# xmed-lab/NEURONS

Hardware: AMD Instinct MI355X
Metric: denoising frames/sec, 16f x 256^2 clip, 50 DDIM steps (higher is better)
Workload: dtype bf16; 1 GPU; BASELINE config 2: 1 clip(s) per call, (1,4,16,32,32) latent, 50 DDIM steps, CFG 8.5 (batch 2), SparseCtrl + temporal U-Net per step, random-init weights; clips_per_gpu=5, ddim_steps=50, hip_graph=True, output_finite=True, attention=bf16

## Files before the change

neurons_amd/csrc/engine.hip:

```cpp
#include "common.h"
#include "../../include/neurons_amd.h"

#include <cmath>
#include <cstdio>
#include <cstdlib>
#include <cstring>
#include <functional>
#include <map>
#include <memory>
#include <stdexcept>
#include <string>
#include <vector>

extern "C" {
int nr_launch_igemm(const NrGemmParams* pp, float* workspace, hipStream_t stream);
size_t nr_igemm_workspace_bytes(const NrGemmParams* pp);
size_t nr_lin160_stream_bytes(int N, int K);
int nr_lin160_eligible(const NrGemmParams* pp);
int nr_lin160_panel_rule(int Mp, int N, int K);
size_t nr_lin128q_stream_bytes(int N, int K);
int nr_launch_lin128q_w_pack(const bf16* w, int N, int K, bf16* stream, hipStream_t s);
int nr_launch_lin160_w_pack(const bf16* w, int N, int K, bf16* stream, hipStream_t s);
int nr_launch_lin160(const NrGemmParams* pp, const bf16* stream, hipStream_t s);
int nr_gn_workspace_floats(int nimg, int hw, int groups, int* pix_per_blk_out, int* nchunk_out);
int nr_launch_groupnorm(NrGnParams* pp, hipStream_t stream);
int nr_launch_layernorm(const bf16* x, int ldx, bf16* out, int ldo, int M, int C, const float* gamma, const float* beta,
                        float eps, const float* pe, int pe_hw, int pe_F, hipStream_t stream);
int nr_launch_attention(const NrAttnParams* pp, hipStream_t stream);
int nr_launch_conv_in_small(const float* s0, const float* s1, int c0, int c1, int src_batch, int nimg, int F, int H, int W,
                            const float* wT, const float* bias, const float* addend, int Cout, bf16* out, float in_scale,
                            float in_shift, hipStream_t stream);
int nr_launch_clip_embed(const int* ids, const float* tok, const float* pos, bf16* out, int M, int L, int C, int vocab,
                         hipStream_t stream);
int nr_launch_bf16_to_f32(const bf16* a, float* out, long long n, hipStream_t stream);
int nr_launch_gaussian_sample(const float* moments, const float* noise, float* out, int n, int zc, int hw, float scale,
                              hipStream_t stream);
int nr_launch_post_quant(const float* z, float scale, const float* Q, const float* qb, float* out, int nimg, int C, int hw,
                         hipStream_t stream);
int nr_launch_softmax_rows(const float* S, bf16* P, int rows, int L, float scale, hipStream_t stream);
int nr_launch_conv_out_small(const bf16* x, int Cin, int nimg, int F, int H, int W, const bf16* w, const float* bias,
                             int Cout, float* out, float out_mul, float out_add, int clamp01, hipStream_t stream);
int nr_launch_timestep_sincos(const float* t, int M, int dim, float* out, hipStream_t stream);
int nr_launch_linear_small(const float* x, int M, int K, const bf16* W, const float* b, int N, int in_act, int out_act,
                           float* y, const float* addend, hipStream_t stream);
int nr_launch_edm_cfg_euler(const float* net, const float* x, float* x_out, long long total, float scale, float sigma_q,
                            float sigma, float sigma_next, hipStream_t stream);
int nr_launch_cfg_combine(const float* eps, float* out, long long total, float guidance, hipStream_t stream);
int nr_launch_cfg_ddim_step(const float* eps, const float* x, float* x_out, long long total, float guidance, int do_cfg,
                            float sqrt_at, float sqrt_1mat, float sqrt_ap, float sqrt_1map, hipStream_t stream);
int nr_launch_add_bf16(const bf16* a, const bf16* b, bf16* out, long long n, hipStream_t stream);
int nr_launch_prior_p_sample(const float* pred, const float* pred_null, const float* x, const float* noise, float* x_out, float* x_start_out,
                             long long total, float cond_scale, int mode, int clamp, float sqrt_ac, float sqrt_1mac, float sqrt_recip_ac,
                             float sqrt_recipm1_ac, float coef1, float coef2, float sigma, hipStream_t stream);
int nr_launch_f32_to_bf16(const float* a, bf16* out, long long n, hipStream_t stream);
int nr_launch_add_bf16_multi(const NrAddMulti* p, hipStream_t stream);
int nr_launch_frame_gather(const bf16* src, bf16* dst, int B, int Fs, int Fd, long long frame_elems, const int* map, hipStream_t stream);
int nr_launch_ncfhw_to_nhwc(const float* src, bf16* dst, int B, int C, int F, int HW, hipStream_t stream);
int nr_launch_nhwc_to_ncfhw(const bf16* src, float* dst, int B, int C, int F, int HW, hipStream_t stream);
int nr_groupnorm_launches(const NrGnParams* p);
int nr_launch_fold_linear_pair(const float* w2, const float* w1, const float* b2, const float* b1, int C, int J, bf16* wc, float* bc,
                               hipStream_t stream);
int nr_smallm_eligible(const NrGemmParams* pp);
int nr_launch_smallm_w_pack(const void* w, void* out, int N, int K, hipStream_t stream);
size_t nr_xattn_wstream_bytes(void);
size_t nr_xattn_kvstream_bytes(int nctx);
int nr_xattn_fused_eligible(int C, int heads, int Lk, int hw, long long rows);
int nr_launch_xattn_w_pack(const bf16* wq, const bf16* wo, bf16* stream, hipStream_t s);
int nr_launch_xattn_kv_pack(const bf16* kv, int ldkv, int Lk, int nctx, bf16* stream, hipStream_t s);
int nr_launch_xattn_fused(bf16* t, int nimg, int hw, int img_per_ctx, int nctx, int Lk, const bf16* wstream, const bf16* kvstream, const float* gamma,
// ... 2785 lines not shown
}

extern "C" nr_status nr_op_gemm_ex(nr_stream stream, const void* a, int32_t lda, const void* w, const float* bias, const float* ln_c,
                                   float ln_eps, const float* rowvec, int32_t rowvec_div, int32_t rowvec_mod, int32_t rowvec_ld,
                                   const void* res, int32_t ldr, void* out, int32_t ldo, int32_t M, int32_t N, int32_t K, int32_t geglu,
                                   int32_t act, float out_scale) {
  NR_TRY
  NrGemmParams p;
  std::memset(&p, 0, sizeof(p));
  p.a0 = (const bf16*)a; p.c0 = K; p.lda0 = lda; p.H = p.W = p.OH = p.OW = 1; p.ksize = 1; p.stride = 1;
  p.w = (const bf16*)w; p.M = M; p.N = N; p.K = K; p.bias = bias; p.res = (const bf16*)res; p.ldr = ldr;
  p.out = (bf16*)out; p.ldo = ldo; p.out_scale = out_scale; p.geglu = geglu; p.act = act;
  p.rowvec = rowvec; p.rowvec_div = rowvec_div > 0 ? rowvec_div : 1; p.rowvec_mod = rowvec_mod; p.rowvec_ld = rowvec_ld;
  p.ln_c = ln_c; p.ln_eps = ln_eps;
  op_fragmajor(p, (hipStream_t)stream);
  LAUNCH_OK(nr_launch_igemm(&p, ln_c ? nullptr : op_workspace(p), (hipStream_t)stream));
  NR_CATCH
}

extern "C" nr_status nr_op_conv3x3(nr_stream stream, const void* x0, int32_t c0, const void* x1, int32_t c1, int32_t nimg,
                                   int32_t H, int32_t W, int32_t stride, int32_t ups, const void* w, const float* bias,
                                   const float* rowvec, int32_t rowvec_div, const void* res, void* out, int32_t Cout) {
  NR_TRY
  NrGemmParams p;
  std::memset(&p, 0, sizeof(p));
  p.a0 = (const bf16*)x0; p.c0 = c0; p.lda0 = c0; p.a1 = (const bf16*)x1; p.c1 = x1 ? c1 : 0; p.lda1 = c1;
  p.H = H; p.W = W;
  int OH = H, OW = W;
  if (ups) { OH *= 2; OW *= 2; }
  if (stride == 2) { OH = (OH - 1) / 2 + 1; OW = (OW - 1) / 2 + 1; }
  p.OH = OH; p.OW = OW; p.ksize = 3; p.stride = stride; p.ups = ups;
  p.w = (const bf16*)w; p.M = nimg * OH * OW; p.N = Cout; p.K = 9 * (p.c0 + p.c1);
  p.bias = bias; p.rowvec = rowvec; p.rowvec_div = rowvec_div > 0 ? rowvec_div : 1; p.rowvec_ld = Cout;
  p.res = (const bf16*)res; p.ldr = Cout; p.out = (bf16*)out; p.ldo = Cout; p.out_scale = 1.f;
  LAUNCH_OK(nr_launch_igemm(&p, op_workspace(p), (hipStream_t)stream));
  NR_CATCH
}

extern "C" nr_status nr_op_conv3x3_tap_inner(nr_stream stream, const void* x0, int32_t c0, int32_t nimg, int32_t H, int32_t W, const void* w,
                                             const float* bias, const float* rowvec, int32_t rowvec_div, const void* res, void* out,
                                             int32_t Cout) {
  NR_TRY
  NrGemmParams p;
  std::memset(&p, 0, sizeof(p));
  p.a0 = (const bf16*)x0; p.c0 = c0; p.lda0 = c0;
  p.H = H; p.W = W; p.OH = H; p.OW = W; p.ksize = 3; p.stride = 1; p.tap_inner = 1;
  p.w = (const bf16*)w; p.M = nimg * H * W; p.N = Cout; p.K = 9 * c0;
  p.bias = bias; p.rowvec = rowvec; p.rowvec_div = rowvec_div > 0 ? rowvec_div : 1; p.rowvec_ld = Cout;
  p.res = (const bf16*)res; p.ldr = Cout; p.out = (bf16*)out; p.ldo = Cout; p.out_scale = 1.f;
  LAUNCH_OK(nr_launch_igemm(&p, op_workspace(p), (hipStream_t)stream));
  NR_CATCH
}

extern "C" nr_status nr_op_groupnorm(nr_stream stream, const void* x0, int32_t c0, const void* x1, int32_t c1, int32_t nimg,
                                     int32_t hw, int32_t groups, const float* gamma, const float* beta, float eps,
                                     int32_t silu, float* partial_ws, void* out) {
  NR_TRY
  NrGnParams p;
  std::memset(&p, 0, sizeof(p));
  p.x0 = (const bf16*)x0; p.c0 = c0; p.ld0 = c0; p.x1 = (const bf16*)x1; p.c1 = x1 ? c1 : 0; p.ld1 = c1;
  p.nimg = nimg; p.hw = hw; p.groups = groups; p.partial = partial_ws; p.gamma = gamma; p.beta = beta; p.eps = eps;
  p.silu = silu; p.out = (bf16*)out; p.ldo = p.c0 + p.c1;
  LAUNCH_OK(nr_launch_groupnorm(&p, (hipStream_t)stream));
  NR_CATCH
}

extern "C" nr_status nr_op_layernorm(nr_stream stream, const void* x, void* out, int32_t M, int32_t C, const float* gamma,
                                     const float* beta, float eps, const float* pe, int32_t pe_hw, int32_t pe_F) {
  NR_TRY
  LAUNCH_OK(nr_launch_layernorm((const bf16*)x, C, (bf16*)out, C, M, C, gamma, beta, eps, pe, pe_hw > 0 ? pe_hw : 1,
                                pe_F > 0 ? pe_F : 1, (hipStream_t)stream));
  NR_CATCH
}

extern "C" nr_status nr_op_attention(nr_stream stream, int32_t mode, const void* qp, const void* kvp, void* outp,
                                     int32_t nimg, int32_t L, int32_t Lk, int32_t C, int32_t heads, int32_t frames,
                                     int32_t kv_div) {
  NR_TRY
  NrAttnParams p;
  std::memset(&p, 0, sizeof(p));
  const bf16* q = (const bf16*)qp; const bf16* kv = (const bf16*)kvp;
  const int fp8_flag = (mode & 8) ? 1 : 0;
  mode &= 7;
  p.heads = heads; p.d = C / heads; p.scale = 1.0f / std::sqrt((float)p.d); p.out = (bf16*)outp;
  if (mode == 0) {
    const int ld = 3 * C;
    p.q = q; p.k = q + C; p.v = q + 2 * C; p.nbatch = nimg; p.Lq = L; p.Lk = L; p.inner = 1; p.kv_inner = 1; p.kv_div = 1;
    p.q_outer = (long long)L * ld; p.q_seq = ld; p.kv_outer = p.q_outer; p.kv_seq = ld;
    p.o_outer = (long long)L * C; p.o_seq = C;
  } else if (mode == 1) {
    p.q = q; p.k = kv; p.v = kv + C; p.nbatch = nimg; p.Lq = L; p.Lk = Lk; p.inner = 1; p.kv_inner = 1; p.kv_div = kv_div;
    p.q_outer = (long long)L * C; p.q_seq = C; p.kv_outer = (long long)Lk * 2 * C; p.kv_seq = 2 * C;
    p.o_outer = (long long)L * C; p.o_seq = C;
  } else if (mode == 2) {
    const int ld = 3 * C, hw = L, F = frames;
    p.q = q; p.k = q + C; p.v = q + 2 * C; p.nbatch = (nimg / F) * hw; p.Lq = F; p.Lk = F; p.inner = hw; p.kv_inner = hw; p.kv_div = 1;
    p.q_outer = (long long)F * hw * ld; p.q_inner_stride = ld; p.q_seq = (long long)hw * ld;
    p.kv_outer = p.q_outer; p.kv_inner_stride = ld; p.kv_seq = p.q_seq;
    p.o_outer = (long long)F * hw * C; p.o_inner_stride = C; p.o_seq = (long long)hw * C;
  } else throw NrError(NR_ERR_ARG, "bad attention mode");
  p.fp8 = fp8_flag;
  LAUNCH_OK(nr_launch_attention(&p, (hipStream_t)stream));
  NR_CATCH
}

extern "C" nr_status nr_op_ff_fused(nr_stream stream, const void* t_dev, const void* x_dev, void* out_dev, int32_t M, int32_t C,
// ... 109 lines not shown
```

neurons_amd/csrc/gemm.hip:

```cpp
#include "common.h"
#include <cstdio>
#include <cstdlib>

namespace {

__device__ __attribute__((aligned(16))) const unsigned int nr_zero16[4] = {0u, 0u, 0u, 0u};

typedef const __attribute__((address_space(1))) void* gptr_t;
typedef __attribute__((address_space(3))) void* lptr_t;

__device__ __forceinline__ void glds16_asm(const void* src, unsigned lds_wave_base) {
  asm volatile("s_mov_b32 m0, %1\n\ts_nop 0\n\tglobal_load_lds_dwordx4 %0, off" : : "v"(src), "s"(lds_wave_base) : "memory", "m0");
}
__device__ __forceinline__ void glds16_builtin(const void* src, void* lds_wave_base) {
  __builtin_amdgcn_global_load_lds((gptr_t)src, (lptr_t)lds_wave_base, 16, 0, 0);
}
__device__ __forceinline__ unsigned lds_addr(const void* p) {
  return __builtin_amdgcn_readfirstlane((unsigned)(unsigned long long)(lptr_t)p);
}

template <int N> __device__ __forceinline__ void wait_vmcnt() {
  if constexpr (N == 0) asm volatile("s_waitcnt vmcnt(0)" ::: "memory");
  else if constexpr (N <= 63) asm volatile("s_waitcnt vmcnt(%0)" ::"n"(N) : "memory");
  else asm volatile("s_waitcnt vmcnt(0)" ::: "memory");
// ... 593 lines not shown
        hipLaunchKernelGGL((igemm_bf16_kernel<BM, BN, NS, WGM, WGN, false, true, true>), dim3(grid), dim3(64 * WGM * WGN), shm, stream, p, splitk, partial, m_fast);
      else
        hipLaunchKernelGGL((igemm_bf16_kernel<BM, BN, NS, WGM, WGN, false, false, true>), dim3(grid), dim3(64 * WGM * WGN), shm, stream, p, splitk, partial, m_fast);
      return 0;
    }
  }
  if (nk_slice >= adma_min)
    hipLaunchKernelGGL((igemm_bf16_kernel<BM, BN, NS, WGM, WGN, false, true>), dim3(grid), dim3(64 * WGM * WGN), shm, stream, p, splitk,
                       partial, m_fast);
  else
    hipLaunchKernelGGL((igemm_bf16_kernel<BM, BN, NS, WGM, WGN, false, false>), dim3(grid), dim3(64 * WGM * WGN), shm, stream, p, splitk,
                       partial, m_fast);
  return 0;
}

template <int BM, int BN, int WGM, int WGN>
int launch_tile(const NrGemmParams& p, unsigned grid, const Plan& pl, float* partial, int m_fast, hipStream_t stream) {
  constexpr size_t STAGE = (size_t)(BM + BN) * 64 * sizeof(bf16);
  constexpr bool FITS4 = 4 * STAGE <= 160 * 1024;
  if (pl.stages <= 2) return launch_cfg<BM, BN, 2, WGM, WGN>(p, grid, pl.splitk, partial, m_fast, stream);
  if (pl.stages == 3 || !FITS4) return launch_cfg<BM, BN, 3, WGM, WGN>(p, grid, pl.splitk, partial, m_fast, stream);
  if (pl.stages <= 4 || BM * BN > 64 * 64) return launch_cfg<BM, BN, 4, WGM, WGN>(p, grid, pl.splitk, partial, m_fast, stream);
  if (pl.stages <= 6) return launch_cfg<BM, BN, 6, WGM, WGN>(p, grid, pl.splitk, partial, m_fast, stream);
  return launch_cfg<BM, BN, 8, WGM, WGN>(p, grid, pl.splitk, partial, m_fast, stream);
}

void apply_override(const NrGemmParams& p, Plan& pl, int& m_fast) {
  const char* e = getenv("NR_IGEMM_FORCE");
  if (!e) return;
  if (const char* f = getenv("NR_IGEMM_FORCE_MAXM")) if (p.M > atoi(f)) return;
  if (const char* f = getenv("NR_IGEMM_FORCE_MINM")) if (p.M < atoi(f)) return;
  if (const char* f = getenv("NR_IGEMM_FORCE_KS")) if (p.ksize != atoi(f)) return;
  if (const char* f = getenv("NR_IGEMM_FORCE_N")) if (p.N != atoi(f)) return;
  if (const char* f = getenv("NR_IGEMM_FORCE_K")) if (p.K != atoi(f)) return;
  int bm = -1, bn = -1, sk = -1, st = -1, ord = -1, wv = -1;
  sscanf(e, "%d,%d,%d,%d,%d,%d", &bm, &bn, &sk, &st, &ord, &wv);
  if (bm > 0 && bn > 0) {
    const bool ok = (bm == 128 && (bn == 160 || bn == 128 || bn == 64)) || (bm == 64 && (bn == 64 || bn == 32 || bn == 160)) || (bm == 256 && (bn == 128 || bn == 160));
    if (ok && !(p.geglu && ((bn == 160 && !(bm == 128 && wv == 41)) || bn == 32))) { pl.bm = bm; pl.bn = bn; }
  }
  if (wv == 4 || wv == 8) pl.waves = wv;
  if (pl.bm == 256 && pl.bn == 128 && wv != 4) pl.waves = 8;
  if (pl.bn == 160 || pl.bm == 64) pl.waves = 4;
  if (wv == 41 && pl.bm == 128 && pl.bn == 160) pl.waves = 41;
  if (sk > 0 && !p.geglu) { const int nk = p.K / 64; pl.splitk = sk > nk ? nk : sk; }
  if (st >= 2 && st <= 8) pl.stages = st;
  if (ord >= 0) m_fast = ord;
}

}

extern "C" int nr_rowpanel_eligible(const NrGemmParams* pp);
extern "C" int nr_launch_rowpanel(const NrGemmParams* pp, hipStream_t stream);
extern "C" int nr_g8p_plan(const NrGemmParams* pp);
extern "C" int nr_launch_g8p(const NrGemmParams* pp, int m_fast, hipStream_t stream);
extern "C" int nr_smallm_eligible(const NrGemmParams* pp);
extern "C" int nr_launch_smallm(const NrGemmParams* pp, hipStream_t stream);

extern "C" size_t nr_igemm_workspace_bytes(const NrGemmParams* pp) {
  if (pp->out_f32 || pp->ln_c) return 0;
  if (nr_rowpanel_eligible(pp)) return 0;
  if (pp->w_fm) return 0;
  if (nr_g8p_plan(pp)) return 0;
  Plan pl = choose_plan(plan_view(*pp));
  int mf = 0;
  apply_override(*pp, pl, mf);
  return pl.splitk > 1 ? (size_t)pl.splitk * pp->M * pp->N * sizeof(float) : 0;
}

extern "C" int nr_launch_igemm(const NrGemmParams* pp, float* workspace, hipStream_t stream) {
  const NrGemmParams& p = *pp;
  const int Cin = p.c0 + p.c1;
  if (p.K == p.ksize * p.ksize * Cin && nr_rowpanel_eligible(pp)) return nr_launch_rowpanel(pp, stream);
  if (p.w_fm) return nr_launch_smallm(pp, stream);
  if (const int nt8 = nr_g8p_plan(pp)) {
    const double w_e = (double)p.N * p.K;
    const double a_e = (double)p.M * Cin;
    int mf = w_e > a_e ? 1 : 0;
    const int ntm_ = (p.M + 255) / 256, ntn_ = (p.N + 64 * nt8 - 1) / (64 * nt8);
    if (ntm_ >= 8 && ntn_ >= 4 && w_e >= 3.0e6) mf = 8;
    return nr_launch_g8p(pp, mf, stream);
  }
  if (p.K % 64 != 0 || Cin % 64 != 0 || p.N % 32 != 0) return 1;
  if (p.a1 && (p.c0 % 64 != 0)) return 2;
  if (p.K != p.ksize * p.ksize * Cin) return 3;
  if (p.ksize != 1 && p.ksize != 3) return 4;
  if (p.tap_inner && (p.ksize != 3 || p.stride != 1 || p.ups || p.pad_tl0 || p.a1)) return 5;
  Plan pl = choose_plan(plan_view(p));
  const double w_elems = (double)p.N * p.K;
  const double a_elems = (double)p.M * Cin * (p.ksize == 3 ? (p.stride == 2 ? 4.0 : (p.ups ? 0.25 : 1.0)) : 1.0);
  int m_fast = w_elems > a_elems ? 1 : 0;
  {
    static const bool grouped = !(getenv("NR_IGEMM_GROUPED") && getenv("NR_IGEMM_GROUPED")[0] == '0');
    const int ntm_ = (p.M + pl.bm - 1) / pl.bm, ntn_ = (p.N + pl.bn - 1) / pl.bn;
    static const double grouped_minw = getenv("NR_IGEMM_GROUPED_MINW") ? atof(getenv("NR_IGEMM_GROUPED_MINW")) : 3.0e6;
    if (grouped && ntm_ >= 8 && ntn_ >= 4 && w_elems >= grouped_minw) m_fast = 8;
  }
  apply_override(p, pl, m_fast);
  if (p.ln_c) {
    if (p.ksize != 1 || p.a1 || p.out_f32) return 8;
    pl.splitk = 1;
    if (pl.bn == 32) pl.bn = 64;
    const bool t64x160 = pl.bm == 64 && pl.bn == 160;
    if (!(pl.stages == 4 && (pl.bm * pl.bn <= 64 * 64 || (pl.bm == 128 && pl.bn == 64))) && pl.waves != 41 && !(t64x160 && pl.stages <= 3)) pl.stages = 2;
    if (pl.bm > 128) { pl.bm = 128; pl.bn = 128; pl.waves = 8; }
    if (pl.bn > 128 && !(pl.bm == 128 && pl.bn == 160 && pl.waves == 41) && !t64x160) { pl.bm = 128; pl.bn = 128; pl.waves = 8; }
    if (pl.waves == 41 && pl.stages > 4) pl.stages = 4;
  }
  if (p.out_f32) {
    if (p.geglu) return 7;
    pl.splitk = 1;
  }
  if (pl.splitk > 1 && !workspace) return 6;
  float* partial = p.out_f32 ? p.out_f32 : (pl.splitk > 1 ? workspace : nullptr);
  const unsigned grid = (unsigned)(((p.M + pl.bm - 1) / pl.bm) * ((p.N + pl.bn - 1) / pl.bn) * pl.splitk);
  int rc;
  if (pl.bm == 256 && pl.bn == 160) rc = launch_tile<256, 160, 2, 2>(p, grid, pl, partial, m_fast, stream);
  else if (pl.bm == 256 && pl.waves == 4) rc = launch_tile<256, 128, 2, 2>(p, grid, pl, partial, m_fast, stream);
  else if (pl.bm == 256) rc = launch_tile<256, 128, 4, 2>(p, grid, pl, partial, m_fast, stream);
  else if (pl.bm == 128 && pl.bn == 160 && pl.waves == 41)
    rc = pl.stages <= 3 ? launch_cfg<128, 160, 3, 4, 1>(p, grid, pl.splitk, partial, m_fast, stream)
                        : launch_cfg<128, 160, 4, 4, 1>(p, grid, pl.splitk, partial, m_fast, stream);
  else if (pl.bm == 128 && pl.bn == 160) rc = launch_tile<128, 160, 2, 2>(p, grid, pl, partial, m_fast, stream);
  else if (pl.bm == 128 && pl.bn == 128 && pl.waves == 8) rc = launch_tile<128, 128, 2, 4>(p, grid, pl, partial, m_fast, stream);
  else if (pl.bm == 128 && pl.bn == 128) rc = launch_tile<128, 128, 2, 2>(p, grid, pl, partial, m_fast, stream);
  else if (pl.bm == 128 && pl.bn == 64 && pl.waves == 8) rc = launch_tile<128, 64, 4, 2>(p, grid, pl, partial, m_fast, stream);
  else if (pl.bm == 128 && pl.bn == 64) rc = launch_tile<128, 64, 2, 2>(p, grid, pl, partial, m_fast, stream);
  else if (pl.bm == 64 && pl.bn == 160) rc = launch_tile<64, 160, 2, 2>(p, grid, pl, partial, m_fast, stream);
  else if (pl.bm == 64 && pl.bn == 32) rc = launch_tile<64, 32, 2, 2>(p, grid, pl, partial, m_fast, stream);
  else if (pl.bm == 64 && pl.bn == 64) rc = launch_tile<64, 64, 2, 2>(p, grid, pl, partial, m_fast, stream);
  else rc = 9;
  if (rc) return rc;
  if (pl.splitk > 1) {
    const long long total = (long long)p.M * (p.N / 4);
// ... 16 lines not shown
```

neurons_amd/csrc/gemm8p.hip:

```cpp
#include "common.h"
#include <cstdlib>

namespace {

__device__ __attribute__((aligned(16))) const unsigned int g8p_zero16[4] = {0u, 0u, 0u, 0u};
typedef __attribute__((address_space(3))) void* lptr_t;

__device__ __forceinline__ void glds16(const void* src, unsigned lds_wave_base) {
  asm volatile("s_mov_b32 m0, %1\n\ts_nop 0\n\tglobal_load_lds_dwordx4 %0, off" : : "v"(src), "s"(lds_wave_base) : "memory", "m0");
}
template <int N> __device__ __forceinline__ void wait_vm() { asm volatile("s_waitcnt vmcnt(%0)" ::"n"(N) : "memory"); }

__device__ __forceinline__ int fdiv_small(int a, int d) {
  int q = (int)((float)a * __builtin_amdgcn_rcpf((float)d));
  const int r = a - q * d;
  q += (r >= d ? 1 : 0) - (r < 0 ? 1 : 0);
  return q;
}
__device__ __forceinline__ size_t rowvec_row(const NrGemmParams& p, int m) {
  int r = m / p.rowvec_div;
  if (p.rowvec_mod) r %= p.rowvec_mod;
  return (size_t)r * p.rowvec_ld;
}

constexpr int G8_BM = 256, G8_BK = 64;

template <int NT, bool TAPI, int NPH = 4>
__global__ __launch_bounds__(512, 2) void g8p_kernel(NrGemmParams p_arg, int m_fast) {
  const NrGemmParams p = nr_pin_params(p_arg);
  m_fast = nr_pin(m_fast);
  constexpr int BN = 64 * NT, WN = 16 * NT;
  constexpr int A_BYTES = G8_BM * 128, B_BYTES = BN * 128, STAGE = A_BYTES + B_BYTES;
  static_assert(NPH == 4 || (NPH == 2 && NT <= 4), "phases per k-tile");
  extern __shared__ __attribute__((aligned(16))) char smem[];

  const int tid = threadIdx.x;
  const int lane = tid & 63;
  const int wave = __builtin_amdgcn_readfirstlane(tid >> 6);
  const int g = wave >> 2, wn = wave & 3;
  const int ntn = (p.N + BN - 1) / BN, ntm = (p.M + G8_BM - 1) / G8_BM;
  int bid;
  {
    const int nwg = gridDim.x, orig = blockIdx.x;
    const int q = nwg >> 3, r = nwg & 7, xcd = orig & 7, local = orig >> 3;
    bid = (xcd < r ? xcd * (q + 1) : r * (q + 1) + (xcd - r) * q) + local;
  }
  int bm, bn;
  if (m_fast >= 2) {
    const int G = m_fast;
    const int band = fdiv_small(bid, G * ntn);
    const int first = band * G;
    const int gsz = min(G, ntm - first);
    const int r = bid - band * G * ntn;
    bn = fdiv_small(r, gsz);
    bm = first + r - bn * gsz;
  } else if (m_fast) { bn = fdiv_small(bid, ntm); bm = bid - bn * ntm; } else { bm = fdiv_small(bid, ntn); bn = bid - bm * ntn; }
  const int m0 = bm * G8_BM, n0 = bn * BN;

  const int lr = lane >> 3, lp = lane & 7;
  const unsigned lchunk_b = (unsigned)((lp ^ lr) << 4);
  const char* zsrc = reinterpret_cast<const char*>(g8p_zero16);

  unsigned a_off[4];
  unsigned a_msk = 0, a_msk3 = 0;
  int a_m[4];
#pragma unroll
  for (int j = 0; j < 4; ++j) {
    const int m = m0 + 8 * (16 * g + 4 * wn + j) + lr;
    const bool ok = m < p.M;
    a_m[j] = ok ? m : 0;
    if constexpr (TAPI) {
      const int ohw = p.OH * p.OW;
      const int n = fdiv_small(a_m[j], ohw);
      const int r = a_m[j] - n * ohw;
      const int oy = fdiv_small(r, p.OW), ox = r - oy * p.OW;
      a_off[j] = (unsigned)((((size_t)n * p.H + oy) * p.W + ox) * (size_t)p.lda0 * sizeof(bf16)) + lchunk_b;
      unsigned msk = 0;
#pragma unroll
      for (int t = 0; t < 9; ++t) {
        const int iy = oy + t / 3 - 1, ix = ox + t % 3 - 1;
        if (ok && iy >= 0 && iy < p.H && ix >= 0 && ix < p.W) msk |= 1u << t;
      }
      if (j < 3) a_msk |= msk << (9 * j);
      else a_msk3 = msk;
    } else {
      a_off[j] = (unsigned)((size_t)a_m[j] * (size_t)p.lda0 * sizeof(bf16)) + lchunk_b;
      if (ok) a_msk |= 1u << j;
    }
  }
  unsigned w_off[NT];
  unsigned w_msk = 0;
#pragma unroll
  for (int j = 0; j < NT; ++j) {
    const int n = n0 + 8 * (NT * wave + j) + lr;
    const bool ok = n < p.N;
    w_off[j] = (unsigned)((size_t)(ok ? n : 0) * (size_t)p.K * sizeof(bf16)) + lchunk_b;
    if (ok) w_msk |= 1u << j;
  }

  const int nk = p.K / G8_BK;
  const unsigned lds0 = __builtin_amdgcn_readfirstlane((unsigned)(unsigned long long)(lptr_t)smem);
  const unsigned lds_a = lds0 + (unsigned)((16 * g + 4 * wn) * 1024);
  const unsigned lds_w = lds0 + (unsigned)A_BYTES + (unsigned)(NT * wave * 1024);

  auto a_base = [&](int kt, int& tap) -> const char* {
    if constexpr (TAPI) {
      const int c64 = kt / 9;
      tap = kt - 9 * c64;
      const int ky = tap / 3, kx = tap - 3 * ky;
      const long long delta = ((long long)(ky - 1) * p.W + (kx - 1)) * p.lda0 * (long long)sizeof(bf16);
      return reinterpret_cast<const char*>(p.a0 + c64 * G8_BK) + delta;
    } else {
      tap = 0;
      const int c = kt * G8_BK;
      return c < p.c0 ? reinterpret_cast<const char*>(p.a0 + c) : reinterpret_cast<const char*>(p.a1 + (c - p.c0));
    }
  };
  int a_src = 0;
  auto a_select_source = [&](int kt) {
    if constexpr (!TAPI) {
      const int want = (p.c1 > 0 && kt * G8_BK >= p.c0) ? 1 : 0;
      if (want != a_src) {
        a_src = want;
        const int ld = want ? p.lda1 : p.lda0;
#pragma unroll
        for (int j = 0; j < 4; ++j) a_off[j] = (unsigned)((size_t)a_m[j] * (size_t)ld * sizeof(bf16)) + lchunk_b;
      }
    }
  };
  auto issue_a = [&](const char* base, int tap, int stage, int j) {
    bool ok;
    if constexpr (TAPI) ok = ((j < 3 ? (a_msk >> (9 * j)) : a_msk3) >> tap) & 1u;
    else ok = (a_msk >> j) & 1u;
    const char* src = ok ? base + a_off[j] : zsrc;
    glds16(src, lds_a + (unsigned)(stage * STAGE + j * 1024));
  };
  auto issue_w = [&](int kt, int stage, int j) {
    const char* base = reinterpret_cast<const char*>(p.w) + (size_t)kt * (G8_BK * sizeof(bf16));
    const char* src = ((w_msk >> j) & 1u) ? base + w_off[j] : zsrc;
    glds16(src, lds_w + (unsigned)(stage * STAGE + j * 1024));
  };

  f32x4 acc[NT][8];
#pragma unroll
  for (int i = 0; i < NT; ++i)
#pragma unroll
    for (int j = 0; j < 8; ++j) acc[i][j] = f32x4{0.f, 0.f, 0.f, 0.f};

  const int fr = lane & 15, fg = lane >> 4;
  const unsigned frag0 = (unsigned)(fr * 128 + ((fg ^ (fr & 7)) << 4));
  const unsigned xrow = (unsigned)(g * 128 * 128), wrow = (unsigned)(A_BYTES + wn * WN * 128);

  {
    int tap;
    a_select_source(0);
    const char* ab = a_base(0, tap);
#pragma unroll
    for (int j = 0; j < 4; ++j) issue_a(ab, tap, 0, j);
#pragma unroll
    for (int j = 0; j < NT; ++j) issue_w(0, 0, j);
    if (nk > 1) {
#pragma unroll
      for (int j = 0; j < NT; ++j) issue_w(1, 1, j);
    }
    wait_vm<0>();
    __builtin_amdgcn_s_barrier();
  }
  if (g == 1) __builtin_amdgcn_s_barrier();

  constexpr int MPP = 8 / NPH;
  constexpr int APP = 4 / (NPH / 2);
  constexpr int WPP = (NT + NPH / 2 - 1) / (NPH / 2);
  constexpr int W_BEFORE_LAST = WPP * (NPH / 2 - 1);
  bf16x8 wf[2][NT], xf[2][MPP];
  for (int t = 0; t < nk; ++t) {
    const int st = t & 1;
    const char* sbase = smem + st * STAGE;
    const bool has1 = t + 1 < nk, has2 = t + 2 < nk;
    int tap1 = 0;
    const char* ab1 = nullptr;
    if (has1) { a_select_source(t + 1); ab1 = a_base(t + 1, tap1); }
#pragma unroll
    for (int ph = 0; ph < NPH; ++ph) {
      if (ph == 0) {
#pragma unroll
        for (int ks = 0; ks < 2; ++ks)
#pragma unroll
          for (int i = 0; i < NT; ++i) wf[ks][i] = *(const bf16x8*)(sbase + wrow + i * 16 * 128 + (frag0 ^ (unsigned)(ks * 64)));
      }
#pragma unroll
      for (int ks = 0; ks < 2; ++ks)
#pragma unroll
        for (int jj = 0; jj < MPP; ++jj) xf[ks][jj] = *(const bf16x8*)(sbase + xrow + (MPP * ph + jj) * 16 * 128 + (frag0 ^ (unsigned)(ks * 64)));
      __builtin_amdgcn_sched_barrier(0);
      if (ph < NPH / 2) {
        if (has1) {
#pragma unroll
          for (int j = 0; j < APP; ++j) issue_a(ab1, tap1, st ^ 1, APP * ph + j);
        }
      } else {
        if (has2) {
#pragma unroll
          for (int j = WPP * (ph - NPH / 2); j < (ph == NPH - 1 ? NT : WPP * (ph - NPH / 2 + 1)); ++j) issue_w(t + 2, st, j);
        }
      }
      if constexpr (NPH == 2) {
        if (ph == 0) asm volatile("s_waitcnt lgkmcnt(0)" ::: "memory");
      }
      __builtin_amdgcn_sched_barrier(0);
      __builtin_amdgcn_s_barrier();
      __builtin_amdgcn_sched_barrier(0);
      __builtin_amdgcn_s_setprio(1);
#pragma unroll
      for (int ks = 0; ks < 2; ++ks)
#pragma unroll
        for (int jj = 0; jj < MPP; ++jj)
#pragma unroll
          for (int i = 0; i < NT; ++i) {
            acc[i][MPP * ph + jj] = __builtin_amdgcn_mfma_f32_16x16x32_bf16(wf[ks][i], xf[ks][jj], acc[i][MPP * ph + jj], 0, 0, 0);
          }
      __builtin_amdgcn_s_setprio(0);
      __builtin_amdgcn_sched_barrier(0);
      if (ph == NPH - 2 && has1) { if (has2) wait_vm<4 + W_BEFORE_LAST>(); else wait_vm<4>(); }
      if (ph == NPH - 1 && has1) { if (has2) wait_vm<NT>(); else wait_vm<0>(); }
      __builtin_amdgcn_s_barrier();
      __builtin_amdgcn_sched_barrier(0);
    }
  }
  if (g == 0) __builtin_amdgcn_s_barrier();

  constexpr int RT = NT <= 4 ? 4 : 2;
  static_assert((size_t)2 * RT * 16 * BN * sizeof(float) <= (size_t)2 * STAGE, "epilogue tile exceeds the LDS ring");
  float* sC = reinterpret_cast<float*>(smem);
  const int bno = p.geglu ? BN / 2 : BN;
  const int c8n = bno >> 3;
  const int nout = p.geglu ? p.N / 2 : p.N;
  const int nb0 = p.geglu ? n0 / 2 : n0;
#pragma unroll
  for (int r = 0; r < 8 / RT; ++r) {
    __syncthreads();
#pragma unroll
    for (int jj = 0; jj < RT; ++jj) {
      const int j = r * RT + jj;
      const int row = (g * RT + jj) * 16 + fr;
      if (!p.geglu) {
#pragma unroll
        for (int i = 0; i < NT; ++i) {
          const int c4 = ((wn * WN + i * 16) >> 2) + fg;
          *(f32x4*)(sC + row * BN + ((c4 ^ (row & 7)) << 2)) = acc[i][j];
        }
      } else {
        if constexpr (NT % 2 == 0) {
#pragma unroll
          for (int i = 0; i < NT; i += 2) {
            const int nv = n0 + wn * WN + i * 16 + 4 * fg;
            f32x4 v = acc[i][j], gt = acc[i + 1][j];
            if (p.bias && nv < p.N) { v += *(const f32x4*)(p.bias + nv); gt += *(const f32x4*)(p.bias + nv + 16); }
            f32x4 o;
#pragma unroll
            for (int e = 0; e < 4; ++e) o[e] = v[e] * gelu_erf_fast(gt[e]);
            const int c4 = (((wn * WN + i * 16) >> 1) >> 2) + fg;
            *(f32x4*)(sC + row * BN + ((c4 ^ (row & 7)) << 2)) = o;
          }
        }
      }
    }
    __syncthreads();
    for (int idx = tid; idx < 2 * RT * 16 * c8n; idx += 512) {
      const int row = idx / c8n, c8 = idx - row * c8n;
      const int gg = row / (RT * 16), lrow = row - gg * (RT * 16);
      const int m = m0 + gg * 128 + r * (RT * 16) + lrow, n = nb0 + c8 * 8;
      if (m >= p.M || n >= nout) continue;
      f32x4 va = *(const f32x4*)(sC + row * BN + (((2 * c8) ^ (row & 7)) << 2));
      f32x4 vb = *(const f32x4*)(sC + row * BN + (((2 * c8 + 1) ^ (row & 7)) << 2));
      if (!p.geglu) {
        if (p.bias) { va += *(const f32x4*)(p.bias + n); vb += *(const f32x4*)(p.bias + n + 4); }
        if (p.rowvec) {
          const float* rv = p.rowvec + rowvec_row(p, m) + n;
          va += *(const f32x4*)rv; vb += *(const f32x4*)(rv + 4);
        }
        va *= p.out_scale; vb *= p.out_scale;
        if (p.act == 1) {
#pragma unroll
          for (int e = 0; e < 4; ++e) { va[e] = quick_gelu_f(va[e]); vb[e] = quick_gelu_f(vb[e]); }
        }
        if (p.res) {
          const bf16x8 rr = *(const bf16x8*)(p.res + (size_t)m * p.ldr + n);
#pragma unroll
          for (int e = 0; e < 4; ++e) { va[e] += (float)rr[e]; vb[e] += (float)rr[4 + e]; }
        }
      }
      bf16x8 o;
#pragma unroll
      for (int e = 0; e < 4; ++e) { o[e] = (bf16)va[e]; o[4 + e] = (bf16)vb[e]; }
      nr_store16(p.out + (size_t)m * p.ldo + n, o);
    }
  }
}

inline bool attr_needed(unsigned long long& mask) {
  int dev = 0;
  (void)hipGetDevice(&dev);
  const unsigned long long bit = 1ull << (dev & 63);
  if (mask & bit) return false;
  mask |= bit;
  return true;
}

template <int NT, bool TAPI, int NPH>
int launch_g8p_n(const NrGemmParams& p, int m_fast, hipStream_t stream) {
  constexpr int BN = 64 * NT;
  constexpr size_t shm = (size_t)2 * (G8_BM + BN) * 128;
  static unsigned long long attr = 0;
  if (attr_needed(attr) &&
      hipFuncSetAttribute((const void*)g8p_kernel<NT, TAPI, NPH>, hipFuncAttributeMaxDynamicSharedMemorySize, (int)shm) != hipSuccess) return 20;
  const unsigned grid = (unsigned)(((p.M + G8_BM - 1) / G8_BM) * ((p.N + BN - 1) / BN));
  hipLaunchKernelGGL((g8p_kernel<NT, TAPI, NPH>), dim3(grid), dim3(512), shm, stream, p, m_fast);
  return 0;
}
static int g8p_phases = -1;
template <int NT, bool TAPI>
int launch_g8p(const NrGemmParams& p, int m_fast, hipStream_t stream) {
  if (g8p_phases < 0) g8p_phases = getenv("NR_G8P_PHASES") ? atoi(getenv("NR_G8P_PHASES")) : 2;
  if constexpr (NT <= 4) { if (g8p_phases == 2) return launch_g8p_n<NT, TAPI, 2>(p, m_fast, stream); }
  return launch_g8p_n<NT, TAPI, 4>(p, m_fast, stream);
}

}

static int g8p_mode = -1;
extern "C" void nr_g8p_set_mode(int mode) { g8p_mode = mode; }
extern "C" void nr_g8p_set_phases(int phases) { g8p_phases = phases == 2 ? 2 : 4; }
extern "C" int nr_g8p_plan(const NrGemmParams* pp) {
  const NrGemmParams& p = *pp;
  if (g8p_mode < 0) g8p_mode = getenv("NR_G8P") ? atoi(getenv("NR_G8P")) : 1;
  const int mode = g8p_mode;
  if (!mode) return 0;
  if (p.ln_c || p.out_f32) return 0;
  const int Cin = p.c0 + p.c1;
  if (p.K % 64 != 0 || Cin % 64 != 0 || p.N % 32 != 0 || p.K != p.ksize * p.ksize * Cin) return 0;
  if (p.ksize == 3) { if (!p.tap_inner || p.stride != 1 || p.ups || p.pad_tl0 || p.a1) return 0; }
  else if (p.ksize != 1) return 0;
  if (p.a1 && p.c0 % 64 != 0) return 0;
  if (p.K / 64 < 4) return 0;
  const size_t rows_src = p.ksize == 3 ? (size_t)(p.M / (p.OH * p.OW)) * p.H * p.W : (size_t)p.M;
  if (rows_src * (size_t)p.lda0 * 2 + 4096 >= 0xffffffffull) return 0;
  if (p.a1 && rows_src * (size_t)p.lda1 * 2 + 4096 >= 0xffffffffull) return 0;
  if ((size_t)p.N * p.K * 2 + 4096 >= 0xffffffffull) return 0;
  if (p.lda0 % 8 != 0 || (p.a1 && p.lda1 % 8 != 0) || p.ldo % 8 != 0 || (p.res && p.ldr % 8 != 0)) return 0;
  if (p.rowvec && p.rowvec_ld % 4 != 0) return 0;
  const long long Mp = p.plan_m > 0 && p.plan_m < p.M ? p.plan_m : p.M;
  const long long ntm = (Mp + G8_BM - 1) / G8_BM;
  const int nk = p.K / 64;
  static const int min_tiles = getenv("NR_G8P_MIN_TILES") ? atoi(getenv("NR_G8P_MIN_TILES")) : 200;
  int best = 0;
  double best_score = 0.0;
  for (int nt = 5; nt >= 2; --nt) {
    if (p.geglu && nt % 2) continue;
    if (mode != 2 && nt < 4) continue;
    const int bn = 64 * nt;
    const long long ntn = (p.N + bn - 1) / bn;
    const long long tiles = ntm * ntn;
    if (mode != 2 && tiles < (nk >= 16 ? min_tiles : 512)) continue;
    const double fill = (double)tiles / (double)(((tiles + 255) / 256) * 256);
    const double used = (double)p.N / (double)(ntn * bn) * (double)Mp / (double)(ntm * G8_BM);
    const double width = nt >= 4 ? 1.0 : (nt == 3 ? 0.9 : 0.8);
    const double score = fill * used * width;
    if (score > best_score) { best_score = score; best = nt; }
  }
  if (mode != 2 && best_score < 0.70) return 0;
  static const int geglu_ok = getenv("NR_G8P_GEGLU") ? atoi(getenv("NR_G8P_GEGLU")) : 1;
  if (mode != 2 && p.geglu) {
    const long long tiles = best ? ntm * ((p.N + 64 * best - 1) / (64 * best)) : 0;
    if (!geglu_ok || tiles < 512 || !(nk >= 16 || Mp >= 32768)) return 0;
  }
  return best;
}

extern "C" int nr_launch_g8p(const NrGemmParams* pp, int m_fast, hipStream_t stream) {
  const NrGemmParams& p = *pp;
  const int nt = nr_g8p_plan(pp);
  if (!nt) return 21;
  const bool tapi = p.ksize == 3;
  switch (nt) {
    case 2: return tapi ? launch_g8p<2, true>(p, m_fast, stream) : launch_g8p<2, false>(p, m_fast, stream);
    case 3: return tapi ? launch_g8p<3, true>(p, m_fast, stream) : launch_g8p<3, false>(p, m_fast, stream);
    case 4: return tapi ? launch_g8p<4, true>(p, m_fast, stream) : launch_g8p<4, false>(p, m_fast, stream);
    case 5: return tapi ? launch_g8p<5, true>(p, m_fast, stream) : launch_g8p<5, false>(p, m_fast, stream);
  }
  return 22;
}
```

Baseline: 20.03 frames/s.

## Add split-K mode to g8p GEMM for low-tile 3x3 tap-inner convolutions

Adds a split-K path to the 256-row g8p implicit-GEMM kernel. Each slice covers a contiguous range of k-tiles and writes fp32 partials to workspace, and an existing splitk reduce kernel then applies the epilogue. The planner turns split-K on for 3x3 tap-inner convs with too few tiles to fill the GPU, when K is deep enough, so those convs can use g8p instead of the fallback GEMM. The cost is extra fp32 workspace traffic and one more reduce launch per conv. A planning helper exposes the workspace size to callers.

```diff
diff --git a/neurons_amd/csrc/engine.hip b/neurons_amd/csrc/engine.hip
--- a/neurons_amd/csrc/engine.hip
+++ b/neurons_amd/csrc/engine.hip
@@ -15,6 +15,7 @@
 extern "C" {
 int nr_launch_igemm(const NrGemmParams* pp, float* workspace, hipStream_t stream);
 size_t nr_igemm_workspace_bytes(const NrGemmParams* pp);
+int nr_g8p_plan(const NrGemmParams* pp, int* splitk);
 size_t nr_lin160_stream_bytes(int N, int K);
 int nr_lin160_eligible(const NrGemmParams* pp);
 int nr_lin160_panel_rule(int Mp, int N, int K);
@@ -2906,6 +2907,20 @@
   NR_CATCH
 }
 
+extern "C" int64_t nr_conv3x3_tap_inner_plan(int32_t c0, int32_t nimg, int32_t H, int32_t W, int32_t Cout, int32_t plan_m, int32_t* g8p_nt, int32_t* splitk) {
+  NrGemmParams p;
+  std::memset(&p, 0, sizeof(p));
+  p.a0 = reinterpret_cast<const bf16*>(uintptr_t(16)); p.c0 = c0; p.lda0 = c0;
+  p.H = H; p.W = W; p.OH = H; p.OW = W; p.ksize = 3; p.stride = 1; p.tap_inner = 1;
+  p.w = reinterpret_cast<const bf16*>(uintptr_t(16)); p.M = nimg * H * W; p.N = Cout; p.K = 9 * c0;
+  p.ldr = Cout; p.ldo = Cout; p.out_scale = 1.f; p.plan_m = plan_m;
+  int sk = 1;
+  const int nt = nr_g8p_plan(&p, &sk);
+  if (g8p_nt) *g8p_nt = nt;
+  if (splitk) *splitk = nt ? sk : 0;
+  return (int64_t)nr_igemm_workspace_bytes(&p);
+}
+
 extern "C" nr_status nr_op_groupnorm(nr_stream stream, const void* x0, int32_t c0, const void* x1, int32_t c1, int32_t nimg,
                                      int32_t hw, int32_t groups, const float* gamma, const float* beta, float eps,
                                      int32_t silu, float* partial_ws, void* out) {
diff --git a/neurons_amd/csrc/gemm.hip b/neurons_amd/csrc/gemm.hip
--- a/neurons_amd/csrc/gemm.hip
+++ b/neurons_amd/csrc/gemm.hip
@@ -669,8 +669,8 @@
 
 extern "C" int nr_rowpanel_eligible(const NrGemmParams* pp);
 extern "C" int nr_launch_rowpanel(const NrGemmParams* pp, hipStream_t stream);
-extern "C" int nr_g8p_plan(const NrGemmParams* pp);
-extern "C" int nr_launch_g8p(const NrGemmParams* pp, int m_fast, hipStream_t stream);
+extern "C" int nr_g8p_plan(const NrGemmParams* pp, int* splitk);
+extern "C" int nr_launch_g8p(const NrGemmParams* pp, int m_fast, int splitk, float* partial, hipStream_t stream);
 extern "C" int nr_smallm_eligible(const NrGemmParams* pp);
 extern "C" int nr_launch_smallm(const NrGemmParams* pp, hipStream_t stream);
 
@@ -678,7 +678,8 @@
   if (pp->out_f32 || pp->ln_c) return 0;
   if (nr_rowpanel_eligible(pp)) return 0;
   if (pp->w_fm) return 0;
-  if (nr_g8p_plan(pp)) return 0;
+  int sk8 = 1;
+  if (nr_g8p_plan(pp, &sk8)) return sk8 > 1 ? (size_t)sk8 * pp->M * pp->N * sizeof(float) : 0;
   Plan pl = choose_plan(plan_view(*pp));
   int mf = 0;
   apply_override(*pp, pl, mf);
@@ -690,13 +691,20 @@
   const int Cin = p.c0 + p.c1;
   if (p.K == p.ksize * p.ksize * Cin && nr_rowpanel_eligible(pp)) return nr_launch_rowpanel(pp, stream);
   if (p.w_fm) return nr_launch_smallm(pp, stream);
-  if (const int nt8 = nr_g8p_plan(pp)) {
+  int sk8 = 1;
+  if (const int nt8 = nr_g8p_plan(pp, &sk8)) {
     const double w_e = (double)p.N * p.K;
     const double a_e = (double)p.M * Cin;
     int mf = w_e > a_e ? 1 : 0;
     const int ntm_ = (p.M + 255) / 256, ntn_ = (p.N + 64 * nt8 - 1) / (64 * nt8);
     if (ntm_ >= 8 && ntn_ >= 4 && w_e >= 3.0e6) mf = 8;
-    return nr_launch_g8p(pp, mf, stream);
+    if (sk8 > 1 && !workspace) return 6;
+    if (const int rc = nr_launch_g8p(pp, mf, sk8, sk8 > 1 ? workspace : nullptr, stream)) return rc;
+    if (sk8 > 1) {
+      const long long total = (long long)p.M * (p.N / 4);
+      hipLaunchKernelGGL(splitk_reduce_kernel, dim3((unsigned)((total + 255) / 256)), dim3(256), 0, stream, p, sk8, (const float*)workspace);
+    }
+    return 0;
   }
   if (p.K % 64 != 0 || Cin % 64 != 0 || p.N % 32 != 0) return 1;
   if (p.a1 && (p.c0 % 64 != 0)) return 2;
diff --git a/neurons_amd/csrc/gemm8p.hip b/neurons_amd/csrc/gemm8p.hip
--- a/neurons_amd/csrc/gemm8p.hip
+++ b/neurons_amd/csrc/gemm8p.hip
@@ -26,9 +26,9 @@
 constexpr int G8_BM = 256, G8_BK = 64;
 
 template <int NT, bool TAPI, int NPH = 4>
-__global__ __launch_bounds__(512, 2) void g8p_kernel(NrGemmParams p_arg, int m_fast) {
+__global__ __launch_bounds__(512, 2) void g8p_kernel(NrGemmParams p_arg, int m_fast, int splitk, float* partial) {
   const NrGemmParams p = nr_pin_params(p_arg);
-  m_fast = nr_pin(m_fast);
+  m_fast = nr_pin(m_fast); splitk = nr_pin(splitk); partial = nr_pin(partial);
   constexpr int BN = 64 * NT, WN = 16 * NT;
   constexpr int A_BYTES = G8_BM * 128, B_BYTES = BN * 128, STAGE = A_BYTES + B_BYTES;
   static_assert(NPH == 4 || (NPH == 2 && NT <= 4), "phases per k-tile");
@@ -45,6 +45,8 @@
     const int q = nwg >> 3, r = nwg & 7, xcd = orig & 7, local = orig >> 3;
     bid = (xcd < r ? xcd * (q + 1) : r * (q + 1) + (xcd - r) * q) + local;
   }
+  const int slice = splitk > 1 ? fdiv_small(bid, ntn * ntm) : 0;
+  bid -= slice * ntn * ntm;
   int bm, bn;
   if (m_fast >= 2) {
     const int G = m_fast;
@@ -99,6 +101,8 @@
   }
 
   const int nk = p.K / G8_BK;
+  const int kb = splitk > 1 ? fdiv_small(nk * slice, splitk) : 0;
+  const int ke = splitk > 1 ? fdiv_small(nk * (slice + 1), splitk) : nk;
   const unsigned lds0 = __builtin_amdgcn_readfirstlane((unsigned)(unsigned long long)(lptr_t)smem);
   const unsigned lds_a = lds0 + (unsigned)((16 * g + 4 * wn) * 1024);
   const unsigned lds_w = lds0 + (unsigned)A_BYTES + (unsigned)(NT * wave * 1024);
@@ -153,15 +157,15 @@
 
   {
     int tap;
-    a_select_source(0);
-    const char* ab = a_base(0, tap);
+    a_select_source(kb);
+    const char* ab = a_base(kb, tap);
 #pragma unroll
     for (int j = 0; j < 4; ++j) issue_a(ab, tap, 0, j);
 #pragma unroll
-    for (int j = 0; j < NT; ++j) issue_w(0, 0, j);
-    if (nk > 1) {
-#pragma unroll
-      for (int j = 0; j < NT; ++j) issue_w(1, 1, j);
+    for (int j = 0; j < NT; ++j) issue_w(kb, 0, j);
+    if (kb + 1 < ke) {
+#pragma unroll
+      for (int j = 0; j < NT; ++j) issue_w(kb + 1, 1, j);
     }
     wait_vm<0>();
     __builtin_amdgcn_s_barrier();
@@ -173,10 +177,10 @@
   constexpr int WPP = (NT + NPH / 2 - 1) / (NPH / 2);
   constexpr int W_BEFORE_LAST = WPP * (NPH / 2 - 1);
   bf16x8 wf[2][NT], xf[2][MPP];
-  for (int t = 0; t < nk; ++t) {
-    const int st = t & 1;
+  for (int t = kb; t < ke; ++t) {
+    const int st = (t - kb) & 1;
     const char* sbase = smem + st * STAGE;
-    const bool has1 = t + 1 < nk, has2 = t + 2 < nk;
+    const bool has1 = t + 1 < ke, has2 = t + 2 < ke;
     int tap1 = 0;
     const char* ab1 = nullptr;
     if (has1) { a_select_source(t + 1); ab1 = a_base(t + 1, tap1); }
@@ -273,6 +277,12 @@
       if (m >= p.M || n >= nout) continue;
       f32x4 va = *(const f32x4*)(sC + row * BN + (((2 * c8) ^ (row & 7)) << 2));
       f32x4 vb = *(const f32x4*)(sC + row * BN + (((2 * c8 + 1) ^ (row & 7)) << 2));
+      if (partial) {
+        float* dst = partial + ((size_t)slice * p.M + m) * p.N + n;
+        nr_store16f(dst, va);
+        nr_store16f(dst + 4, vb);
+        continue;
+      }
       if (!p.geglu) {
         if (p.bias) { va += *(const f32x4*)(p.bias + n); vb += *(const f32x4*)(p.bias + n + 4); }
         if (p.rowvec) {
@@ -308,22 +318,22 @@
 }
 
 template <int NT, bool TAPI, int NPH>
-int launch_g8p_n(const NrGemmParams& p, int m_fast, hipStream_t stream) {
+int launch_g8p_n(const NrGemmParams& p, int m_fast, int splitk, float* partial, hipStream_t stream) {
   constexpr int BN = 64 * NT;
   constexpr size_t shm = (size_t)2 * (G8_BM + BN) * 128;
   static unsigned long long attr = 0;
   if (attr_needed(attr) &&
       hipFuncSetAttribute((const void*)g8p_kernel<NT, TAPI, NPH>, hipFuncAttributeMaxDynamicSharedMemorySize, (int)shm) != hipSuccess) return 20;
-  const unsigned grid = (unsigned)(((p.M + G8_BM - 1) / G8_BM) * ((p.N + BN - 1) / BN));
-  hipLaunchKernelGGL((g8p_kernel<NT, TAPI, NPH>), dim3(grid), dim3(512), shm, stream, p, m_fast);
+  const unsigned grid = (unsigned)(((p.M + G8_BM - 1) / G8_BM) * ((p.N + BN - 1) / BN) * splitk);
+  hipLaunchKernelGGL((g8p_kernel<NT, TAPI, NPH>), dim3(grid), dim3(512), shm, stream, p, m_fast, splitk, partial);
   return 0;
 }
 static int g8p_phases = -1;
 template <int NT, bool TAPI>
-int launch_g8p(const NrGemmParams& p, int m_fast, hipStream_t stream) {
+int launch_g8p(const NrGemmParams& p, int m_fast, int splitk, float* partial, hipStream_t stream) {
   if (g8p_phases < 0) g8p_phases = getenv("NR_G8P_PHASES") ? atoi(getenv("NR_G8P_PHASES")) : 2;
-  if constexpr (NT <= 4) { if (g8p_phases == 2) return launch_g8p_n<NT, TAPI, 2>(p, m_fast, stream); }
-  return launch_g8p_n<NT, TAPI, 4>(p, m_fast, stream);
+  if constexpr (NT <= 4) { if (g8p_phases == 2) return launch_g8p_n<NT, TAPI, 2>(p, m_fast, splitk, partial, stream); }
+  return launch_g8p_n<NT, TAPI, 4>(p, m_fast, splitk, partial, stream);
 }
 
 }
@@ -331,8 +341,9 @@
 static int g8p_mode = -1;
 extern "C" void nr_g8p_set_mode(int mode) { g8p_mode = mode; }
 extern "C" void nr_g8p_set_phases(int phases) { g8p_phases = phases == 2 ? 2 : 4; }
-extern "C" int nr_g8p_plan(const NrGemmParams* pp) {
+extern "C" int nr_g8p_plan(const NrGemmParams* pp, int* splitk_out) {
   const NrGemmParams& p = *pp;
+  if (splitk_out) *splitk_out = 1;
   if (g8p_mode < 0) g8p_mode = getenv("NR_G8P") ? atoi(getenv("NR_G8P")) : 1;
   const int mode = g8p_mode;
   if (!mode) return 0;
@@ -352,6 +363,8 @@
   const long long Mp = p.plan_m > 0 && p.plan_m < p.M ? p.plan_m : p.M;
   const long long ntm = (Mp + G8_BM - 1) / G8_BM;
   const int nk = p.K / 64;
+  const char* sk_env = getenv("NR_G8P_SPLITK");
+  const int sk_force = sk_env ? atoi(sk_env) : 1;
   static const int min_tiles = getenv("NR_G8P_MIN_TILES") ? atoi(getenv("NR_G8P_MIN_TILES")) : 200;
   int best = 0;
   double best_score = 0.0;
@@ -368,6 +381,31 @@
     const double score = fill * used * width;
     if (score > best_score) { best_score = score; best = nt; }
   }
+  if (mode == 2 && best && !p.geglu && sk_force >= 2) {
+    if (splitk_out) *splitk_out = sk_force < nk ? sk_force : nk;
+    return best;
+  }
+  static const int sk_mink = getenv("NR_G8P_SPLITK_MINK") ? atoi(getenv("NR_G8P_SPLITK_MINK")) : 40;
+  if (mode != 2 && !best && !p.geglu && p.ksize == 3 && sk_force != 0) {
+    int best_sk = 1;
+    for (int nt = 5; nt >= 4; --nt) {
+      const int bn = 64 * nt;
+      const long long ntn = (p.N + bn - 1) / bn;
+      const long long tiles = ntm * ntn;
+      const double used = (double)p.N / (double)(ntn * bn) * (double)Mp / (double)(ntm * G8_BM);
+      for (int sk = 2; sk <= (sk_force >= 2 ? nk : 16); ++sk) {
+        if (sk_force >= 2 && sk != sk_force) continue;
+        if (sk_force < 2 && nk / sk < sk_mink) break;
+        const long long wg = tiles * sk;
+        if (sk_force < 2 && wg % 256 != 0) continue;
+        const double score = (double)wg / (double)(((wg + 255) / 256) * 256) * used;
+        if (score > best_score) { best_score = score; best = nt; best_sk = sk; }
+      }
+    }
+    if (!best || (sk_force < 2 && best_score < 0.70)) return 0;
+    if (splitk_out) *splitk_out = best_sk;
+    return best;
+  }
   if (mode != 2 && best_score < 0.70) return 0;
   static const int geglu_ok = getenv("NR_G8P_GEGLU") ? atoi(getenv("NR_G8P_GEGLU")) : 1;
   if (mode != 2 && p.geglu) {
@@ -377,16 +415,18 @@
   return best;
 }
 
-extern "C" int nr_launch_g8p(const NrGemmParams* pp, int m_fast, hipStream_t stream) {
+extern "C" int nr_launch_g8p(const NrGemmParams* pp, int m_fast, int splitk, float* partial, hipStream_t stream) {
   const NrGemmParams& p = *pp;
-  const int nt = nr_g8p_plan(pp);
+  const int nt = nr_g8p_plan(pp, nullptr);
   if (!nt) return 21;
+  if (splitk < 1 || (splitk > 1 && (!partial || p.geglu || splitk > p.K / 64))) return 23;
+  if (splitk == 1) partial = nullptr;
   const bool tapi = p.ksize == 3;
   switch (nt) {
-    case 2: return tapi ? launch_g8p<2, true>(p, m_fast, stream) : launch_g8p<2, false>(p, m_fast, stream);
-    case 3: return tapi ? launch_g8p<3, true>(p, m_fast, stream) : launch_g8p<3, false>(p, m_fast, stream);
-    case 4: return tapi ? launch_g8p<4, true>(p, m_fast, stream) : launch_g8p<4, false>(p, m_fast, stream);
-    case 5: return tapi ? launch_g8p<5, true>(p, m_fast, stream) : launch_g8p<5, false>(p, m_fast, stream);
+    case 2: return tapi ? launch_g8p<2, true>(p, m_fast, splitk, partial, stream) : launch_g8p<2, false>(p, m_fast, splitk, partial, stream);
+    case 3: return tapi ? launch_g8p<3, true>(p, m_fast, splitk, partial, stream) : launch_g8p<3, false>(p, m_fast, splitk, partial, stream);
+    case 4: return tapi ? launch_g8p<4, true>(p, m_fast, splitk, partial, stream) : launch_g8p<4, false>(p, m_fast, splitk, partial, stream);
+    case 5: return tapi ? launch_g8p<5, true>(p, m_fast, splitk, partial, stream) : launch_g8p<5, false>(p, m_fast, splitk, partial, stream);
   }
   return 22;
 }
```

New measurement: 20.02 frames/s, median of 2. No clear change (-0.0%).
